# ShiveshM/GolemFlavor

Measured on AMD Instinct MI355X. Metric: walker-lnprob evals/sec (Gaussian llh, 100 walkers) at 1/2/4/8 MI355X, higher is better.
Workload: dtype f64

## Files before the change

### golemflavor_amd/csrc/gf_device.hpp

```cpp
#pragma once
#include <hip/hip_runtime.h>
#include <stdint.h>

#include "gf_consts.h"
#include "gf_elements.hpp"

#define GF_WAVE 64
#define GF_BLOCK 256
#define GF_WAVES_PER_BLOCK (GF_BLOCK / GF_WAVE)

#ifdef GF_COS_LITERALS
#define GF_COSC(c) nullptr
#else
#define GF_COSC(c) (c).cosc
#endif

namespace gfdev {

constexpr int ST_OK = 0, ST_OUT_OF_PRIOR = 1, ST_NON_UNITARY = 2, ST_NAN = 3;
constexpr int MODE_PRIOR_ONLY = 0, MODE_SM_GAUSS = 1, MODE_BSM_GAUSS = 2;
constexpr int MODE_BSM_BINNED = 3;
constexpr int MODE_BSM_TABLE = 4;

__device__ __forceinline__ double gf_inf() { return __longlong_as_double(0x7ff0000000000000LL); }
__device__ __forceinline__ double gf_nan() { return __longlong_as_double(0x7ff8000000000000LL); }


__device__ __forceinline__ double fast_sqrt(double x) { return gfel::el_sqrt(x); }

__device__ __forceinline__ double fast_rcp(double x)
{
    double r = __builtin_amdgcn_rcp(x);
    r = fma(fma(-x, r, 1.0), r, r);
    r = fma(fma(-x, r, 1.0), r, r);
    return r;
}

static __device__ __attribute__((noinline)) void sincos_cold(double x, double* sn, double* cs) { sincos(x, sn, cs); }

__device__ __forceinline__ void fast_sincos(double x, double* sn, double* cs)
{
    gfel::sincos_cw(x, sn, cs);
}

__device__ __forceinline__ double fast_cos(double x)
{
    double s, c;
    fast_sincos(x, &s, &c);
    return c;
}

static __device__ __attribute__((noinline)) double cos_general(double x) { return fast_cos(x); }

__device__ __forceinline__ double fast_cos_phase(double x, const double* k = nullptr)
{
    const double u = fabs(x - 3.141592653589793) - 1.5707963267948966;
    if (!(fabs(u) <= 1.5707963277948966)) return cos_general(x);
    const double z = u * u;
    double q;
    if (k) {
        q = fma(z, k[0], k[1]);
        q = fma(z, q, k[2]);
        q = fma(z, q, k[3]);
        q = fma(z, q, k[4]);
        q = fma(z, q, k[5]);
        q = fma(z, q, k[6]);
        q = fma(z, q, k[7]);
    } else {
        q = fma(z, 2.7117413873509064e-15, -7.641995277350052e-13);
        q = fma(z, q, 1.605889634387573e-10);
        q = fma(z, q, -2.505210587009456e-08);
        q = fma(z, q, 2.75573191979119e-06);
        q = fma(z, q, -0.00019841269841110079);
        q = fma(z, q, 0.008333333333332799);
        q = fma(z, q, -0.16666666666666657);
    }
    return fma(u * z, q, u);
}

__constant__ double GF_KTAB[26] = {
    2.7117413873509064e-15, -7.641995277350052e-13, 1.605889634387573e-10, -2.505210587009456e-08,
    2.75573191979119e-06, -0.00019841269841110079, 0.008333333333332799, -0.16666666666666657,
    4.695137892341541e-14, -1.1468837412893726e-11, 2.0876733673699156e-09, -2.755731905787651e-07,
    2.4801587300891894e-05, -0.0013888888888887252, 0.04166666666666665, -0.5,
    3.47933107596021167570e-05, 7.91534994289814532176e-04, -4.00555345006794114027e-02, 2.01212532134862925881e-01,
    -3.25565818622400915405e-01, 1.66666666666666657415e-01,
    7.70381505559019352791e-02, -6.88283971605453293030e-01, 2.02094576023350569471e+00, -2.40339491173441421878e+00};

__device__ __forceinline__ void sincos_small(double u, double* sn, double* cs)
{
    const double* k = GF_KTAB;
    const double z = u * u;
    double q = fma(z, k[0], k[1]);
    q = fma(z, q, k[2]);
    q = fma(z, q, k[3]);
    q = fma(z, q, k[4]);
    q = fma(z, q, k[5]);
    q = fma(z, q, k[6]);
    q = fma(z, q, k[7]);
    *sn = fma(u * z, q, u);
    double c = fma(z, k[8], k[9]);
    c = fma(z, c, k[10]);
    c = fma(z, c, k[11]);
    c = fma(z, c, k[12]);
    c = fma(z, c, k[13]);
    c = fma(z, c, k[14]);
    c = fma(z, c, k[15]);
    *cs = fma(z, c, 1.0);
}

__device__ __forceinline__ double fast_acos(double x)
{
    const double* k = GF_KTAB + 16;
    const double ax = fabs(x);
    const bool big = ax > 0.5;
    const double z = big ? fma(-0.5, ax, 0.5) : x * x;
    const double s = big ? fast_sqrt(z) : ax;
    double p = fma(z, k[0], k[1]);
    p = fma(z, p, k[2]);
    p = fma(z, p, k[3]);
    p = fma(z, p, k[4]);
    p = fma(z, p, k[5]);
    double q = fma(z, k[6], k[7]);
    q = fma(z, q, k[8]);
    q = fma(z, q, k[9]);
    q = fma(z, q, 1.0);
    const double r = (z * p) * fast_rcp(q);
    const double as = fma(s, r, s);
    const double a = big ? as + as : 1.5707963267948966 - as;
    return x < 0.0 ? 3.141592653589793 - a : a;
}

__device__ __forceinline__ double fast_acos_clamped(double x)
{
    const double* k = GF_KTAB + 16;
    const double ax = fabs(x);
    const bool big = ax > 0.5;
    const double z = big ? fmax(fma(-0.5, ax, 0.5), 0.0) : x * x;
    const double s = big ? fast_sqrt(z) : ax;
    double p = fma(z, k[0], k[1]);
    p = fma(z, p, k[2]);
    p = fma(z, p, k[3]);
    p = fma(z, p, k[4]);
// ... 6 lines not shown
    const double as = fma(s, r, s);
    const double a = big ? as + as : 1.5707963267948966 - as;
    return x < 0.0 ? 3.141592653589793 - a : a;
}

static __device__ __attribute__((noinline)) double pow10_cold(double x) { return pow(10.0, x); }
#ifdef GF_POW_LIBRARY
__device__ __forceinline__ double pow10_scale(double x) { return pow10_cold(x); }
#else
__constant__ double GF_P10TAB[18] = {
    3.321928094887362, 0.30102999560767785, 5.630334806675098e-11,
    1.3508629476223687e-06, 8.213412535439387e-06, 4.6371516642572196e-05, 0.00024166672554424694,
    0.0011544997789984348, 0.00501392883377544, 0.019597694626478524, 0.06808936507443707, 0.2069958486968681,
    0.5393829291955814, 1.171255148912267, 2.034678592293476, 2.650949055239199, 2.302585092994046, 1.0};
__device__ __forceinline__ double pow10_scale(double x)
{
    if (!(fabs(x) < 300.0)) return pow10_cold(x);
    const double* k = GF_P10TAB;
    const double n = rint(x * k[0]);
    double r = fma(-n, k[1], x);
    r = fma(-n, k[2], r);
    double p = k[3];
#pragma unroll
    for (int j = 4; j < 18; ++j) p = fma(p, r, k[j]);
    return ldexp(p, (int)n);
}
#endif

template <int NDIM>
__device__ __forceinline__ void stage_theta(const double* __restrict__ theta, int layout, int64_t n,
                                            int64_t w0, int ndim_rt, double* tile, int lane, int64_t n_stage = -1)
{
    const int ndim = NDIM ? NDIM : ndim_rt;
    const int64_t nlim = n_stage < 0 ? n : n_stage;
    const int64_t rows = (nlim - w0 < GF_WAVE) ? (nlim - w0) : GF_WAVE;
    if (layout == 0) {
        const int64_t count = rows * ndim;
        const double* src = theta + w0 * ndim;
        const int nvec = (GF_WAVE * ndim + 1) / 2;
#pragma unroll
        for (int j = 0; j < (NDIM ? (NDIM + 1) / 2 : (GF_MAX_DIM / 2)); ++j) {
            const int v = j * GF_WAVE + lane;
            if (!NDIM && v >= nvec) break;
            const int64_t d = 2 * (int64_t)v;
            if (d + 1 < count) {
                const double2 x = *reinterpret_cast<const double2*>(src + d);
                *reinterpret_cast<double2*>(tile + d) = x;
            } else if (d < count) {
                tile[d] = src[d];
            }
        }
    } else {
        if (lane < rows) {
#pragma unroll
            for (int d = 0; d < (NDIM ? NDIM : GF_MAX_DIM); ++d) {
                if (!NDIM && d >= ndim) break;
                tile[lane * ndim + d] = theta[(int64_t)d * n + w0 + lane];
            }
        }
    }
    __builtin_amdgcn_fence(__ATOMIC_RELEASE, "wavefront");
    __builtin_amdgcn_wave_barrier();
    __builtin_amdgcn_fence(__ATOMIC_ACQUIRE, "wavefront");
}

template <int NDIM>
__device__ __forceinline__ bool lnprior(const GfCommon& c, const double* row, double& lp)
{
    const int ndim = NDIM ? NDIM : c.ndim;
    bool inbox = true;
    double acc = 0.0;
#pragma unroll
    for (int d = 0; d < (NDIM ? NDIM : GF_MAX_DIM); ++d) {
        if (!NDIM && d >= ndim) break;
        const double x = row[d];
        inbox = inbox && (x >= c.lo[d]) && (x <= c.hi[d]);
        const double z = (x - c.loc[d]) * c.inv_sigma[d];
        acc = fma(-0.5 * z, z, acc);
    }
    lp = acc + c.prior_const;
    return inbox;
}

__device__ __forceinline__ void pmns_abs2(double s12_2, double c13_4, double s23_2, double dcp, double p[3][3],
                                          const double* cosc = nullptr)
{
    const double c13_2 = fast_sqrt(c13_4);
    const double s13_2 = 1.0 - c13_2;
    const double c12_2 = 1.0 - s12_2;
    const double c23_2 = 1.0 - s23_2;
    const double a = s12_2 * c23_2, b = c12_2 * s23_2;
    const double e = c12_2 * c23_2, f = s12_2 * s23_2;
    const double j2 = 2.0 * fast_sqrt((a * b) * s13_2) * fast_cos_phase(dcp, cosc);
    p[0][0] = c12_2 * c13_2;
    p[0][1] = s12_2 * c13_2;
    p[0][2] = s13_2;
    p[1][0] = fma(b, s13_2, a) + j2;
    p[1][1] = fma(f, s13_2, e) - j2;
    p[1][2] = s23_2 * c13_2;
}

using gfel::angles_to_fr;

__device__ __forceinline__ void propagate(const double p[3][3], const double src[3], double src_sum, double out[3])
{
    const double inv = fast_rcp(src_sum);
    const double s2 = src[2] * inv;
    const double ds0 = fma(src[0], inv, -s2), ds1 = fma(src[1], inv, -s2);
    const double w0 = fma(ds1, p[1][0], fma(ds0, p[0][0], s2));
    const double w1 = fma(ds1, p[1][1], fma(ds0, p[0][1], s2));
    const double w2 = fma(ds1, p[1][2], fma(ds0, p[0][2], s2));
    const double dw0 = w0 - w2, dw1 = w1 - w2;
    out[0] = fma(p[0][1], dw1, fma(p[0][0], dw0, w2));
    out[1] = fma(p[1][1], dw1, fma(p[1][0], dw0, w2));
    out[2] = (((w0 + w1) + w2) - out[0]) - out[1];
}

static __device__ __attribute__((noinline)) double log_of_exp_band(double x)
{
    const double HI = 744.4400719213812, LO = 4.422444340918698e-14;
    const double t = x + HI;
    const double y = exp(t) * (1.0 + LO);
    const double k = rint(y);
    if (!(k >= 1.0)) return (x != x) ? x : -gf_inf();
    return (log(k) - HI) - LO;
}

__device__ __forceinline__ double log_of_exp(double x, bool live = true)
{
    if (!live || x >= -708.3964185322641) return x;
    return log_of_exp_band(x);
}

__device__ __forceinline__ double gauss_llh(const GfCommon& c, const double fr[3], bool live = true)
{
    const double d0 = fr[0] - c.bf[0];
    const double d1 = fr[1] - c.bf[1];
    const double d2 = fr[2] - c.bf[2];
    const double r2 = fma(d2, d2, fma(d1, d1, d0 * d0));
    const double logpdf = fma(c.gauss_mh, r2, c.gauss_k);
    return log_of_exp(logpdf, live) + c.offset;
}

__device__ __forceinline__ double pick(const double* row, int idx, double fixed)
{
    return idx >= 0 ? row[idx] : fixed;
}

__device__ __forceinline__ void sm_composition(const GfCommon& c, const double* row, double fr[3])
{
    double p[3][3];
    pmns_abs2(pick(row, c.idx_sm[0], c.sm_fixed[0]), pick(row, c.idx_sm[1], c.sm_fixed[1]),
              pick(row, c.idx_sm[2], c.sm_fixed[2]), pick(row, c.idx_sm[3], c.sm_fixed[3]), p);
    double src[3], src_sum;
    if (c.idx_src[0] >= 0) {
        angles_to_fr(row[c.idx_src[0]], row[c.idx_src[1]], src);
        src_sum = (src[0] + src[1]) + src[2];
    } else if (c.idx_src_x >= 0) {
        const double x = row[c.idx_src_x], y = 1.0 - x;
        const double inv = fast_rcp((x + y) + 0.0);
        src[0] = x * inv; src[1] = y * inv; src[2] = 0.0;
        src_sum = (src[0] + src[1]) + src[2];
    } else {
        src[0] = c.src_fixed[0]; src[1] = c.src_fixed[1]; src[2] = c.src_fixed[2];
        src_sum = c.src_fixed_sum;
    }
    propagate(p, src, src_sum, fr);
}


template <int NDIM, int MODE, int SAMPLED, bool WANT_FR>
__device__ __forceinline__ void eval_walker(const GfCommon& c, const double* ctab, const double* row, int ndim_rt,
                                            double& val, double fr[3], int& st)
{
    const int ndim = NDIM ? NDIM : ndim_rt;
    bool inbox = true;
    double acc = 0.0;
#pragma unroll
    for (int d = 0; d < (NDIM ? NDIM : GF_MAX_DIM); ++d) {
        if (!NDIM && d >= ndim) break;
        const double x = row[d];
        const double2 lh = *reinterpret_cast<const double2*>(ctab + 4 * d);
        const double2 ls = *reinterpret_cast<const double2*>(ctab + 4 * d + 2);
        inbox = inbox & (x >= lh.x) & (x <= lh.y);
        const double z = (x - ls.x) * ls.y;
        acc = fma(-0.5 * z, z, acc);
#ifdef GF_DIM_BARRIER
        if ((d % GF_DIM_BARRIER) == GF_DIM_BARRIER - 1) __builtin_amdgcn_sched_barrier(0);
#endif
    }
    const double lp = acc + c.prior_const;
    double v;
    if (MODE == MODE_PRIOR_ONLY) {
        v = lp + c.flat_llh;
        if (WANT_FR) fr[0] = fr[1] = fr[2] = gf_nan();
    } else {
        double f[3];
        if (SAMPLED == 2) {
            double p[3][3], src[3];
            pmns_abs2(row[0], row[1], row[2], row[3], p, GF_COSC(c));
            angles_to_fr(row[4], row[5], src);
            propagate(p, src, (src[0] + src[1]) + src[2], f);
        } else if (SAMPLED == 1) {
            double p[3][3], src[3];
            pmns_abs2(row[c.idx_sm[0]], row[c.idx_sm[1]], row[c.idx_sm[2]], row[c.idx_sm[3]], p, GF_COSC(c));
            angles_to_fr(row[c.idx_src[0]], row[c.idx_src[1]], src);
            propagate(p, src, (src[0] + src[1]) + src[2], f);
        } else {
            sm_composition(c, row, f);
        }
        v = lp + gauss_llh(c, f, inbox);
        if (WANT_FR) {
            fr[0] = inbox ? f[0] : gf_nan(); fr[1] = inbox ? f[1] : gf_nan(); fr[2] = inbox ? f[2] : gf_nan();
        }
    }
    val = inbox ? v : -gf_inf();
    st = inbox ? ((v != v) ? ST_NAN : ST_OK) : ST_OUT_OF_PRIOR;
}


}
```

### golemflavor_amd/csrc/gf_propose.hpp

```cpp
#pragma once
#include <cstdlib>

#include "gf_device.hpp"
#include "gf_bsm_device.hpp"
#include "gf_launch.h"
#include "gf_table.hpp"

namespace {
using namespace gfdev;

__device__ __forceinline__ void philox_block(uint32_t c0, uint32_t c1, uint32_t c2, uint32_t c3, uint32_t k0,
                                             uint32_t k1, uint32_t out[4])
{
#pragma unroll
    for (int r = 0; r < 10; ++r) {
        const uint64_t m0 = (uint64_t)0xD2511F53u * c0;
        const uint64_t m1 = (uint64_t)0xCD9E8D57u * c2;
        const uint32_t n0 = __builtin_amdgcn_bitop3_b32((uint32_t)(m1 >> 32), c1, k0, 0x96);
        const uint32_t n1 = (uint32_t)m1;
        const uint32_t n2 = __builtin_amdgcn_bitop3_b32((uint32_t)(m0 >> 32), c3, k1, 0x96);
        const uint32_t n3 = (uint32_t)m0;
        c0 = n0; c1 = n1; c2 = n2; c3 = n3;
        k0 += 0x9E3779B9u; k1 += 0xBB67AE85u;
    }
    out[0] = c0; out[1] = c1; out[2] = c2; out[3] = c3;
}

template <int NDIM, int MODE, int LPW>
__device__ __forceinline__ double proposal_lnprob(const GfCommon& c, const GfBsm* tb, const double* ctab,
                                                  const double* ttab, const double* row, int ndim, int& st, int sub,
                                                  double* fgrp, unsigned long long& pending, const double* btab = nullptr,
                                                  int tside = 0)
{
    pending = 0ull;
    double val, fr[3];
    if constexpr (MODE == MODE_BSM_TABLE) {
        double lp;
        const bool inbox = lnprior_tab<NDIM>(ctab, row, ndim, c.prior_const, lp);
        asm volatile("" : "+v"(lp));
        val = -gf_inf();
        st = ST_OUT_OF_PRIOR;
        if (inbox) {
            UniAcc acc = {0.0, 0.0, 0ull, 2.0};
            flux_average<UNI_INLINE, LPW>(c, tb, ttab, row, fr, acc, sub, fgrp);
            st = (acc.clear_max < tb->uni_hi) ? ST_OK : ST_NON_UNITARY;
            pending = st == ST_OK ? uni_arbitration_mask(acc.amb, tb) : 0ull;
            val = lp + gftab::lookup(btab, tside, fr[0], fr[1]);
            if (val != val && st == ST_OK) st = ST_NAN;
        }
    } else if constexpr (MODE == MODE_BSM_BINNED || MODE == MODE_BSM_GAUSS) {
        static_assert(MODE != MODE_BSM_BINNED || LPW == 1, "the binned likelihood runs one lane per point");
        double lp;
        const bool inbox = lnprior_tab<NDIM>(ctab, row, ndim, c.prior_const, lp);
        asm volatile("" : "+v"(lp));
        val = -gf_inf();
        st = ST_OUT_OF_PRIOR;
        if (inbox) {
            UniAcc acc = {0.0, 0.0, 0ull, 2.0};
            double lnl = 0.0;
            if constexpr (MODE == MODE_BSM_BINNED) lnl = binned_llh<UNI_INLINE>(c, tb, ttab, btab, row, acc) + c.offset;
            else flux_average<UNI_INLINE, LPW>(c, tb, ttab, row, fr, acc, sub, fgrp);
            st = (acc.clear_max < tb->uni_hi) ? ST_OK : ST_NON_UNITARY;
            pending = st == ST_OK ? uni_arbitration_mask(acc.amb, tb) : 0ull;
            if constexpr (MODE != MODE_BSM_BINNED) lnl = gauss_llh(c, fr);
            val = lp + lnl;
            if (val != val && st == ST_OK) st = ST_NAN;
        }
    } else {
        eval_walker<NDIM, MODE, 0, false>(c, ctab, row, ndim, val, fr, st);
    }
    return val;
}

__device__ __forceinline__ void park_row(double* dst, const double* row, int ndim)
{
    for (int d = 0; d < ndim; ++d) dst[d] = row[d];
}

template <bool WITH_LHS = false>
__device__ __forceinline__ void park_proposal(GfArbQueue* pq, double* pend_rows, int64_t t, const double* row, int ndim, double lnq,
                                              unsigned long long pending, double lhs = 0.0)
{
    double* dst = pend_rows + (size_t)t * GF_PEND_STRIDE;
    park_row(dst, row, ndim);
    dst[GF_MAX_DIM] = lnq;
    if (WITH_LHS) dst[GF_MAX_DIM + 1] = lhs;
    const unsigned int at = atomicAdd(&pq->count, 1u);
    if (at < pq->cap) {
        GfArbItem it;
        it.walker = (unsigned long long)t;
        it.mask = pending;
        pq->items[at] = it;
    } else {
        pq->overflow = 1u;
    }
}

struct GfLpwRule {
    bool with2;
    size_t lds_cap;
    const char* force_env;
};
inline int lanes_per_walker(int mode, int64_t walkers, int nbins_max, int cus, const GfLpwRule& rule)
{
    if (mode != MODE_BSM_GAUSS || nbins_max < 2) return 1;
    const char* force = gf_internal_env(rule.force_env, 0);
    if (force) { const int f = std::atoi(force); if (f == 1 || (f == 2 && rule.with2) || f == 4 || f == 16) return f; }
    const int64_t simds = (int64_t)(cus > 0 ? cus : 256) * 4;
    int best = 1;
    double best_cost = 0.0;
    for (int lpw : {1, 2, 4, 16}) {
        if (lpw == 2 && !rule.with2) continue;
// ... 16 lines not shown
```

### golemflavor_amd/csrc/gf_sampler.hip

```cpp
#include <hip/hip_runtime.h>
#include <stdint.h>

#include <chrono>
#include <cstdio>
#include <cstdlib>
#include <cstring>
#include <cstddef>
#include <memory>
#include <new>

#include "gf_devcache.h"
#include "gf_host.h"
#include "gf_device.hpp"
#include "gf_bsm_device.hpp"
#include "gf_launch.h"
#include "gf_unitarity_teams.hpp"
#include "gf_propose.hpp"
#include "gf_stretch.hpp"

namespace {
using namespace gfdev;


struct StretchArgs {
// ... 102 lines not shown
        }
        s.lnp[wi] = lnq;
        s.naccept[wi] += 1u;
    }
    if (store_now) {
        double* dst = s.chain + (((int64_t)chain * s.nstore_cap + store_index) * s.nwalkers + w) * ndim;
#pragma unroll
        for (int d = 0; d < ND; ++d) {
            if (!NDIM && d >= ndim) break;
            dst[d] = accept ? row[d] : sk[d];
        }
        if (s.lnp_chain)
            s.lnp_chain[((int64_t)chain * s.nstore_cap + store_index) * s.nwalkers + w] = accept ? lnq : lnk;
    }
    }
}

#ifndef GF_STRETCH_WAVES
#define GF_STRETCH_WAVES 2
#endif
template <int NDIM, int MODE, int LPW>
__global__ __launch_bounds__(GF_BLOCK, GF_STRETCH_WAVES) void k_stretch(const GfCommon c, const GfBsm* __restrict__ tb,
                                                          const double* __restrict__ ptab, const StretchArgs s)
{
    const int nhalf = s.nwalkers / 2;
    const int64_t t = (int64_t)blockIdx.x * GF_BLOCK + threadIdx.x;
    const int64_t g = t / LPW;
    const bool valid = g < (int64_t)s.nchains * nhalf;
    const int chain = valid ? (int)(g / nhalf) : 0;
    const int k = valid ? (int)(g - (int64_t)chain * nhalf) : 0;
    if constexpr (MODE == MODE_BSM_BINNED) stretch_body<NDIM, MODE, LPW>(c, tb, ptab, s, chain, k, valid, 0, s.btabs[0]);
    else if constexpr (MODE == MODE_BSM_TABLE) stretch_body<NDIM, MODE, LPW>(c, tb, ptab, s, chain, k, valid, (int)(t % LPW), s.ttabs[0], s.tsides[0]);
    else stretch_body<NDIM, MODE, LPW>(c, tb, ptab, s, chain, k, valid, (int)(t % LPW));
}

template <int NDIM, int MODE, int LPW>
__global__ __launch_bounds__(GF_BLOCK, GF_STRETCH_WAVES) void k_stretch_multi(const StretchArgs s)
{
    const int chain = blockIdx.y;
    const int t = blockIdx.x * GF_BLOCK + threadIdx.x;
    const int k = t / LPW;
    if constexpr (MODE == MODE_BSM_BINNED)
        stretch_body<NDIM, MODE, LPW>(s.commons[chain], s.tbs[chain], s.ptabs[chain], s, chain, k, k < s.nwalkers / 2, 0, s.btabs[chain]);
    else if constexpr (MODE == MODE_BSM_TABLE)
        stretch_body<NDIM, MODE, LPW>(s.commons[chain], s.tbs[chain], s.ptabs[chain], s, chain, k, k < s.nwalkers / 2, t % LPW, s.ttabs[chain],
                                      s.tsides[chain]);
    else stretch_body<NDIM, MODE, LPW>(s.commons[chain], s.tbs[chain], s.ptabs[chain], s, chain, k, k < s.nwalkers / 2, t % LPW);
}

template <int NDIM, int MODE, int LPW>
hipError_t launch_stretch_nml(const GfCommon& c, const GfBsm* tb, const double* ptab, const StretchArgs& a, hipStream_t st)
{
    const size_t lds = LPW > 1 ? (size_t)(GF_BLOCK / LPW) * GF_FGRP_DOUBLES(a.nbins_max, LPW) * sizeof(double) : 0;
    if (a.commons) {
        const dim3 grid((unsigned)(((int64_t)(a.nwalkers / 2) * LPW + GF_BLOCK - 1) / GF_BLOCK), a.nchains);
        hipLaunchKernelGGL((k_stretch_multi<NDIM, MODE, LPW>), grid, dim3(GF_BLOCK), lds, st, a);
    } else {
        const int64_t total = (int64_t)a.nchains * (a.nwalkers / 2) * LPW;
        hipLaunchKernelGGL((k_stretch<NDIM, MODE, LPW>), dim3((unsigned)((total + GF_BLOCK - 1) / GF_BLOCK)), dim3(GF_BLOCK), lds, st,
                           c, tb, ptab, a);
    }
    return hipGetLastError();
}

struct PersistArgs {
    const GfCommon* commons;
    const double* const* ptabs;
    int32_t nmodels;
    int32_t nwalkers;
    double* pos;
    double* lnp;
    uint32_t* naccept;
    double* chain;
    double* lnp_chain;
    int64_t nstore_cap, store_base;
    uint64_t seed, iteration_base;
    int64_t nsteps;
    int32_t thin, store;
    double a;
    const uint64_t* stream_ids;
    int32_t workers;
};

template <int NDIM, int MODE, int MAXT>
__global__ __launch_bounds__(MAXT) void k_stretch_persist(const PersistArgs s)
{
    constexpr int ND = NDIM ? NDIM : GF_MAX_DIM;
    extern __shared__ __attribute__((aligned(16))) double dyn[];
    const int chain = blockIdx.x;
    const GfCommon& c = s.commons[s.nmodels > 1 ? chain : 0];
    const double* __restrict__ ptab = s.ptabs[s.nmodels > 1 ? chain : 0];
    const int ndim = NDIM ? NDIM : c.ndim;
    const int nw = s.nwalkers, nhalf = nw / 2, nt = blockDim.x;
    const int ntw = s.workers > 0 && s.workers < nt ? s.workers : nt;
    const int ntp = nt - ntw;
    const bool producer = (int)threadIdx.x >= ntw;
    double* ctab = dyn;
    double* pos = ctab + GF_MAX_DIM * 4;
    double* lnp = pos + (size_t)nw * ndim;
    double* rows = lnp + nw;
    uint32_t* nacc = reinterpret_cast<uint32_t*>(rows + (size_t)ntw * ndim);
    double* dz = reinterpret_cast<double*>(nacc + ((nw + 1) & ~1));
    double* dlhs = dz + 2 * (size_t)nhalf;
    int* dj = reinterpret_cast<int*>(dlhs + 2 * (size_t)nhalf);
    if (threadIdx.x < GF_MAX_DIM * 4) ctab[threadIdx.x] = ptab[threadIdx.x];
    const int64_t cw = (int64_t)chain * nw;
    for (int i = threadIdx.x; i < nw * ndim; i += nt) pos[i] = s.pos[cw * ndim + i];
    for (int i = threadIdx.x; i < nw; i += nt) { lnp[i] = s.lnp[cw + i]; nacc[i] = s.naccept[cw + i]; }
    double* row = rows + (size_t)(producer ? 0 : threadIdx.x) * ndim;
    const uint64_t gbase = (s.stream_ids ? s.stream_ids[chain] : (uint64_t)chain) * (uint64_t)nhalf;
    auto draw = [&](int k, uint64_t ctr, double& z, int& j, double& lhs) {
        double u3;
        stretch_draw(s.seed, gbase + (uint64_t)k, ctr, nhalf, s.a, z, j, u3);
        lhs = stretch_lhs(z, u3, ndim);
    };
    const uint64_t ctr_first = 2 * s.iteration_base, ctr_end = ctr_first + 2 * (uint64_t)s.nsteps;
    if (producer && s.nsteps > 0)
        for (int k = (int)threadIdx.x - ntw; k < nhalf; k += ntp) {
            double z, lhs; int j;
            draw(k, ctr_first, z, j, lhs);
            dz[k] = z; dlhs[k] = lhs; dj[k] = j;
        }
    __syncthreads();

    for (int64_t step = 0; step < s.nsteps; ++step) {
        const uint64_t iteration = s.iteration_base + (uint64_t)step;
        const bool store_now = s.store != 0 && s.chain != nullptr && (step % s.thin) == 0;
        const int64_t store_index = s.store_base + (step + s.thin - 1) / s.thin;
        for (int half = 0; half < 2; ++half) {
            const int cbase = (1 - half) * nhalf;
            const uint64_t ctr = 2 * iteration + half;
            const size_t buf = (size_t)(half) * nhalf;
            if (producer) {
                if (ctr + 1 < ctr_end)
                    for (int k = (int)threadIdx.x - ntw; k < nhalf; k += ntp) {
                        double z, lhs; int j;
                        draw(k, ctr + 1, z, j, lhs);
                        const size_t nb = (size_t)(1 - half) * nhalf;
                        dz[nb + k] = z; dlhs[nb + k] = lhs; dj[nb + k] = j;
                    }
            } else
            for (int k = threadIdx.x; k < nhalf; k += ntw) {
                const int w = half * nhalf + k;
                double z, lhs; int j;
                if (ntp > 0) { z = dz[buf + k]; lhs = dlhs[buf + k]; j = dj[buf + k]; }
                else draw(k, ctr, z, j, lhs);
                double* sk = pos + (size_t)w * ndim;
                const double* cj = pos + (size_t)(cbase + j) * ndim;
                stretch_row<NDIM>(row, cj, sk, z, ndim);
                int st;
                unsigned long long pending;
                const double lnq = proposal_lnprob<NDIM, MODE, 1>(c, nullptr, ctab, nullptr, row, ndim, st, 0, nullptr, pending);
                const double lnk = lnp[w];
                const bool accept = lhs > lnk - lnq;
                if (accept) {
#pragma unroll
                    for (int d = 0; d < ND; ++d) {
                        if (!NDIM && d >= ndim) break;
                        sk[d] = row[d];
                    }
                    lnp[w] = lnq;
                    nacc[w] += 1u;
                }
                if (store_now) {
                    double* dst = s.chain + (((int64_t)chain * s.nstore_cap + store_index) * nw + w) * ndim;
#pragma unroll
                    for (int d = 0; d < ND; ++d) {
                        if (!NDIM && d >= ndim) break;
                        dst[d] = sk[d];
                    }
                    if (s.lnp_chain) s.lnp_chain[((int64_t)chain * s.nstore_cap + store_index) * nw + w] = lnp[w];
                }
            }
            __syncthreads();
        }
    }
    for (int i = threadIdx.x; i < nw * ndim; i += nt) s.pos[cw * ndim + i] = pos[i];
    for (int i = threadIdx.x; i < nw; i += nt) { s.lnp[cw + i] = lnp[i]; s.naccept[cw + i] = nacc[i]; }
}

inline void persist_geometry(int nwalkers, int ndim, int* threads, size_t* lds, int* workers = nullptr, int nchains = 1, int cus = 256)
{
    const int nhalf = nwalkers / 2;
    int nt = ((nhalf + GF_WAVE - 1) / GF_WAVE) * GF_WAVE;
    if (nt > 512) nt = 512;
    static const bool no_producers = gf_internal_env("GF_SAMPLER_NO_PRODUCERS", 0) != nullptr;
    const size_t base = sizeof(double) * ((size_t)GF_MAX_DIM * 4 + (size_t)nwalkers * ndim + nwalkers + (size_t)nt * ndim) +
                        sizeof(uint32_t) * (size_t)((nwalkers + 1) & ~1);
    const size_t draws = (sizeof(double) * 4 + sizeof(int) * 2) * (size_t)nhalf;
    const bool producers = nt <= 256 && !no_producers && base + draws <= 64 * 1024 && nchains <= 2 * cus;
    const size_t bytes = base + (producers ? draws : 0);
    if (workers) *workers = nt;
    *threads = producers ? 2 * nt : nt;
    *lds = (bytes <= 64 * 1024 && nhalf <= 4 * 1024) ? bytes : 0;
}

template <int NDIM>
hipError_t launch_persist_n(int mode, int nchains, int threads, size_t lds, const PersistArgs& a, hipStream_t st)
{
    if (mode == MODE_PRIOR_ONLY) {
        if (threads <= 256) hipLaunchKernelGGL((k_stretch_persist<NDIM, MODE_PRIOR_ONLY, 256>), dim3(nchains), dim3(threads), lds, st, a);
        else hipLaunchKernelGGL((k_stretch_persist<NDIM, MODE_PRIOR_ONLY, 512>), dim3(nchains), dim3(threads), lds, st, a);
    } else {
        if (threads <= 256) hipLaunchKernelGGL((k_stretch_persist<NDIM, MODE_SM_GAUSS, 256>), dim3(nchains), dim3(threads), lds, st, a);
        else hipLaunchKernelGGL((k_stretch_persist<NDIM, MODE_SM_GAUSS, 512>), dim3(nchains), dim3(threads), lds, st, a);
    }
    return hipGetLastError();
}

hipError_t launch_persist(int mode, int ndim, int nchains, int threads, size_t lds, const PersistArgs& a, hipStream_t st)
{
    switch (ndim) {
    case 4: return launch_persist_n<4>(mode, nchains, threads, lds, a, st);
    case 6: return launch_persist_n<6>(mode, nchains, threads, lds, a, st);
    case 7: return launch_persist_n<7>(mode, nchains, threads, lds, a, st);
    case 12: return launch_persist_n<12>(mode, nchains, threads, lds, a, st);
    default: return launch_persist_n<0>(mode, nchains, threads, lds, a, st);
    }
}

struct ChainArgs {
    const GfCommon* commons;
    const GfBsm* const* tbs;
    const GfBsm* tb;
    const double* const* ptabs;
    int32_t nmodels;
    int32_t nwalkers;
    double* pos;
    double* lnp;
    uint32_t* naccept;
    uint32_t* flags;
    double* pend_rows;
    double* chain;
    double* lnp_chain;
    int64_t nstore_cap, store_base;
    uint64_t seed, iteration_base;
    int64_t run_step_base;
    int32_t nsteps, thin, store;
    double a;
    const uint64_t* stream_ids;
    double* lazy_rows;
    unsigned long long* lazy_mask;
    int32_t lazy_cap;
    unsigned long long* stats;
};

constexpr int CH_BLOCK = 512;
constexpr int CH_WAVES = CH_BLOCK / GF_WAVE;

typedef __attribute__((address_space(3))) double* LdsD;
typedef __attribute__((address_space(3))) unsigned int* LdsU;
typedef __attribute__((address_space(3))) int* LdsI;
typedef __attribute__((address_space(3))) unsigned long long* LdsL;

template <int NDIM>
__device__ __attribute__((noinline)) void chain_propose(const ChainArgs& s, const GfCommon& c, const GfBsm* __restrict__ tb, LdsD ctab_l, LdsD ttab_l,
                                                        LdsD row_l, const int chain, const int k, const int half, const uint64_t iteration,
                                                        const bool store_now, const int64_t store_index, const uint64_t sid, double* my_pend,
                                                        double* lz_rows, unsigned long long* lz_mask, LdsU pk_n, LdsI pk_k, LdsL pk_mask, LdsU lz_n)
{
    constexpr int ND = NDIM ? NDIM : GF_MAX_DIM;
    const double* ctab = (const double*)ctab_l;
    const double* ttab = (const double*)ttab_l;
    double* row = (double*)row_l;
    const int ndim = NDIM ? NDIM : c.ndim;
    const int nw = s.nwalkers, nhalf = nw / 2;
    const int cbase = (1 - half) * nhalf;
    const uint64_t g = sid * (uint64_t)nhalf + (uint64_t)k;
    const int w = half * nhalf + k;
    double z, u3;
    int j;
    stretch_draw(s.seed, g, 2 * iteration + half, nhalf, s.a, z, j, u3);
    const int64_t wi = (int64_t)chain * nw + w;
    const double* sk = s.pos + wi * ndim;
    const double* cj = s.pos + ((int64_t)chain * nw + cbase + j) * ndim;
#pragma unroll
    for (int d = 0; d < ND; ++d) {
        if (!NDIM && d >= ndim) break;
        const double cv = cj[d];
        row[d] = fma(-z, cv - sk[d], cv);
    }
    int st;
    unsigned long long pending;
    const double lnq = proposal_lnprob<NDIM, MODE_BSM_GAUSS, 1>(c, tb, ctab, ttab, row, ndim, st, 0, nullptr, pending);
    const double lnk = s.lnp[wi];
    const double lhs = stretch_lhs(z, u3, ndim);
    bool accept = lhs > lnk - lnq;
    if (pending != 0ull && accept) {
        double* dst = my_pend + (size_t)k * GF_PEND_STRIDE;
        park_row(dst, row, ndim);
        dst[GF_MAX_DIM] = lnq;
        dst[GF_MAX_DIM + 1] = lhs;
        const unsigned int at = atomicAdd((unsigned int*)pk_n, 1u);
        pk_k[at] = k;
        pk_mask[at] = pending;
    } else {
        if (pending != 0ull) {
            const unsigned int at = atomicAdd((unsigned int*)lz_n, 1u);
            park_row(lz_rows + (size_t)at * GF_PEND_STRIDE, row, ndim);
            lz_mask[at] = pending;
        }
// ... 996 lines not shown
    s->steps_since_reset += nsteps;
    s->nstored += nstore;
    return GF_OK;
}

int gf_sampler_sync(gf_sampler* s)
{
    if (!s) return GF_ERR_INVALID_ARG;
    return gf_model_sync(s->model);
}

int gf_sampler_run_to_host(gf_sampler* s, int64_t nsteps, int thin, double* chain, double* lnprob_chain, double* readback_tail_s)
{
    if (!s || !chain || nsteps < 0 || thin < 1) return GF_ERR_INVALID_ARG;
    GF_HIP(hipSetDevice(s->device));
    const int device = s->device;
    void* copy_stream = nullptr;
    int rc = gf_internal_borrow_copy_stream(device, &copy_stream);
    if (rc != GF_OK) return rc;
    HostSink sink;
    sink.chain = chain; sink.lnp = lnprob_chain; sink.total = s->nstored + (nsteps + thin - 1) / thin;
    sink.copy_stream = copy_stream; sink.device = device;
    sink.last_event = sink.t_entry = std::chrono::steady_clock::now();
    if (gf_internal_env("GF_RUN_TO_HOST_NO_PIPE", 0) == nullptr) {
        rc = gf_internal_d2h_pipe_open(device, copy_stream, &sink.pipe);
        if (rc != GF_OK) { gf_internal_return_copy_stream(device, copy_stream); return rc; }
    }
    const bool marks = gf_internal_env("GF_RUN_TO_HOST_NO_MARKS", 0) == nullptr;
    s->sink = marks ? &sink : nullptr;
    rc = gf_sampler_run(s, nsteps, thin, 1);
    hipError_t e = hipSuccess;
    while (rc == GF_OK && e == hipSuccess && s->flight_done < s->flight_enq) e = flight_consume(s, true);
    s->sink = nullptr;
    const hipError_t e2 = hipStreamSynchronize(s->stream);
    auto t_done = marks && s->flight_enq > 0 ? sink.last_event : std::chrono::steady_clock::now();
    if (rc == GF_OK && e == hipSuccess && e2 == hipSuccess && sink.rc == GF_OK) {
        s->sink = &sink;
        (void)sink_copy(s, s->nstored);
        s->sink = nullptr;
    }
    const int rc_pipe = gf_internal_d2h_pipe_close(sink.pipe);
    (void)hipStreamSynchronize((hipStream_t)copy_stream);
    gf_internal_return_copy_stream(device, copy_stream);
    if (rc == GF_OK && sink.rc == GF_OK) sink.rc = rc_pipe;
    if (readback_tail_s) *readback_tail_s = std::chrono::duration<double>(std::chrono::steady_clock::now() - t_done).count();
    for (int i = 0; i < 8; ++i) g_last_run_to_host_times[i] = sink.t[i];
    if (rc != GF_OK) return rc;
    if (sink.rc != GF_OK) return sink.rc;
    if (e == hipSuccess) e = e2;
    if (e != hipSuccess) return gf_hip_fail(e, "gf_sampler_run_to_host");
    return GF_OK;
}

int gf_internal_sampler_chain_stats(gf_sampler* s, unsigned long long* out)
{
    if (!s || !out) return GF_ERR_INVALID_ARG;
    if (!s->d_chain_stats) return GF_ERR_UNSUPPORTED;
    GF_HIP(hipSetDevice(s->device));
    GF_HIP(hipMemcpyAsync(out, s->d_chain_stats, sizeof(unsigned long long) * 8 * (size_t)s->nchains, hipMemcpyDeviceToHost, s->stream));
    GF_HIP(hipStreamSynchronize(s->stream));
    return GF_OK;
}

int gf_internal_run_to_host_times(double out[8])
{
    if (!out) return GF_ERR_INVALID_ARG;
    for (int i = 0; i < 8; ++i) out[i] = g_last_run_to_host_times[i];
    return GF_OK;
}
int gf_internal_run_prologue_times(double out[4])
{
    if (!out) return GF_ERR_INVALID_ARG;
    for (int i = 0; i < 4; ++i) out[i] = g_last_run_prologue[i];
    return GF_OK;
}

int gf_internal_sampler_shape(const gf_sampler* s, double out[3])
{
    if (!s || !out) return GF_ERR_INVALID_ARG;
    out[0] = (double)s->shape; out[1] = s->probe_us[0]; out[2] = s->probe_us[1];
    return GF_OK;
}

int64_t gf_sampler_nstored(const gf_sampler* s) { return s ? s->nstored : -1; }
int64_t gf_sampler_iterations(const gf_sampler* s) { return s ? s->steps_since_reset : -1; }

int gf_internal_sampler_chain_view(const gf_sampler* s, GfChainView* v)
{
    if (!s || !v) return GF_ERR_INVALID_ARG;
    *v = GfChainView{s->device, s->stream, s->cus, s->nchains, s->nwalkers, s->ndim, s->nstored, s->nstore_cap, s->d_chain, s->model, s->models,
                     s->d_lnp_chain, s->seed, s->d_stream_ids};
    return GF_OK;
}

int gf_sampler_get_state(gf_sampler* s, double* pos, double* lnprob)
{
    if (!s) return GF_ERR_INVALID_ARG;
    int rc = gf_model_sync(s->model);
    if (rc != GF_OK) return rc;
    GF_HIP(hipSetDevice(s->device));
    const size_t nw = (size_t)s->nchains * s->nwalkers;
    hipStream_t st = s->stream;
    if (pos) GF_HIP(hipMemcpyAsync(pos, s->d_pos, sizeof(double) * nw * s->ndim, hipMemcpyDeviceToHost, st));
    if (lnprob) GF_HIP(hipMemcpyAsync(lnprob, s->d_lnp, sizeof(double) * nw, hipMemcpyDeviceToHost, st));
    GF_HIP(hipStreamSynchronize(st));
    return GF_OK;
}

int gf_sampler_get_chain(gf_sampler* s, double* chain, double* lnprob_chain, uint32_t* naccepted, uint32_t* nonunitary)
{
    if (!s) return GF_ERR_INVALID_ARG;
    GF_HIP(hipSetDevice(s->device));
    hipStream_t st = s->stream;
    const size_t per = (size_t)s->nwalkers;
    if (s->nstored > 0) {
        const size_t row = sizeof(double) * per * s->ndim, lrow = sizeof(double) * per;
        if (chain) {
            const int rc = gf_internal_d2h_2d(s->device, st, chain, row * s->nstored, s->d_chain, row * s->nstore_cap, row * s->nstored,
                                              (size_t)s->nchains);
            if (rc != GF_OK) return rc;
        }
        if (lnprob_chain) {
            const int rc = gf_internal_d2h_2d(s->device, st, lnprob_chain, lrow * s->nstored, s->d_lnp_chain, lrow * s->nstore_cap,
                                              lrow * s->nstored, (size_t)s->nchains);
            if (rc != GF_OK) return rc;
        }
    }
    if (naccepted)
        GF_HIP(hipMemcpyAsync(naccepted, s->d_naccept, sizeof(uint32_t) * (size_t)s->nchains * per, hipMemcpyDeviceToHost, st));
    if (nonunitary) GF_HIP(hipMemcpyAsync(nonunitary, s->d_flags, sizeof(uint32_t), hipMemcpyDeviceToHost, st));
    GF_HIP(hipStreamSynchronize(st));
    return GF_OK;
}

int gf_sampler_get_chain_device(gf_sampler* s, double* d_chain, double* d_lnprob_chain)
{
    if (!s) return GF_ERR_INVALID_ARG;
    GF_HIP(hipSetDevice(s->device));
    hipStream_t st = s->stream;
    if (s->nstored > 0) {
        const size_t row = sizeof(double) * (size_t)s->nwalkers * s->ndim, lrow = sizeof(double) * (size_t)s->nwalkers;
        if (d_chain)
            GF_HIP(hipMemcpy2DAsync(d_chain, row * s->nstored, s->d_chain, row * s->nstore_cap, row * s->nstored, s->nchains,
                                     hipMemcpyDeviceToDevice, st));
        if (d_lnprob_chain)
            GF_HIP(hipMemcpy2DAsync(d_lnprob_chain, lrow * s->nstored, s->d_lnp_chain, lrow * s->nstore_cap, lrow * s->nstored,
                                     s->nchains, hipMemcpyDeviceToDevice, st));
    }
    GF_HIP(hipStreamSynchronize(st));
    return GF_OK;
}

hipError_t gf_launch_walker_mean(const double* d_chain, int64_t cap, int64_t nstored, int nchains, int nwalkers, int ndim, double* d_mean,
                                 hipStream_t st)
{
    hipError_t e = hipSuccess;
    for (int ch0 = 0; ch0 < nchains && e == hipSuccess; ch0 += 65535) {
        const int nch = nchains - ch0 < 65535 ? nchains - ch0 : 65535;
        hipLaunchKernelGGL(k_walker_mean, dim3((unsigned)nstored, (unsigned)nch), dim3(GF_BLOCK), 0, st,
                           d_chain + (size_t)ch0 * cap * nwalkers * ndim, cap, nstored, nwalkers, ndim, d_mean + (size_t)ch0 * nstored * ndim);
        e = hipGetLastError();
    }
    return e;
}

int gf_sampler_walker_mean(gf_sampler* s, double* mean)
// ... 19 lines not shown
```

Baseline: 106.1 billion.

## Stage persistent-kernel constants in LDS and raise waves-per-EU launch bounds

The persistent stretch kernel now copies the per-chain model constants, seed, output pointers and chain-store bases into a shared-memory struct once per block. The inner loop reads from that struct through templated likelihood helpers, with 32-bit indexing and incremental store counters, and launch bounds request 4 waves per EU for small NDIM. The aim is to cut SGPR/VGPR pressure and 64-bit address arithmetic so more waves can be resident and scalar loads drop. In exchange it uses more LDS per block, risks spills under the tighter register cap, and adds a diagnostic resource-query entry point.

```diff
diff --git a/golemflavor_amd/csrc/gf_device.hpp b/golemflavor_amd/csrc/gf_device.hpp
--- a/golemflavor_amd/csrc/gf_device.hpp
+++ b/golemflavor_amd/csrc/gf_device.hpp
@@ -52,13 +52,14 @@
 
 static __device__ __attribute__((noinline)) double cos_general(double x) { return fast_cos(x); }
 
+template <bool TABLE = false>
 __device__ __forceinline__ double fast_cos_phase(double x, const double* k = nullptr)
 {
     const double u = fabs(x - 3.141592653589793) - 1.5707963267948966;
     if (!(fabs(u) <= 1.5707963277948966)) return cos_general(x);
     const double z = u * u;
     double q;
-    if (k) {
+    if (TABLE || k) {
         q = fma(z, k[0], k[1]);
         q = fma(z, q, k[2]);
         q = fma(z, q, k[3]);
@@ -231,6 +232,7 @@
     return inbox;
 }
 
+template <bool TABLE = false>
 __device__ __forceinline__ void pmns_abs2(double s12_2, double c13_4, double s23_2, double dcp, double p[3][3],
                                           const double* cosc = nullptr)
 {
@@ -240,7 +242,7 @@
     const double c23_2 = 1.0 - s23_2;
     const double a = s12_2 * c23_2, b = c12_2 * s23_2;
     const double e = c12_2 * c23_2, f = s12_2 * s23_2;
-    const double j2 = 2.0 * fast_sqrt((a * b) * s13_2) * fast_cos_phase(dcp, cosc);
+    const double j2 = 2.0 * fast_sqrt((a * b) * s13_2) * fast_cos_phase<TABLE>(dcp, cosc);
     p[0][0] = c12_2 * c13_2;
     p[0][1] = s12_2 * c13_2;
     p[0][2] = s13_2;
@@ -281,7 +283,8 @@
     return log_of_exp_band(x);
 }
 
-__device__ __forceinline__ double gauss_llh(const GfCommon& c, const double fr[3], bool live = true)
+template <class C>
+__device__ __forceinline__ double gauss_llh(const C& c, const double fr[3], bool live = true)
 {
     const double d0 = fr[0] - c.bf[0];
     const double d1 = fr[1] - c.bf[1];
@@ -296,11 +299,23 @@
     return idx >= 0 ? row[idx] : fixed;
 }
 
-__device__ __forceinline__ void sm_composition(const GfCommon& c, const double* row, double fr[3])
+template <class C>
+struct SmCosc {
+    static constexpr bool table = true;
+    static __device__ __forceinline__ const double* of(const C& c) { return c.cosc; }
+};
+template <>
+struct SmCosc<GfCommon> {
+    static constexpr bool table = false;
+    static __device__ __forceinline__ const double* of(const GfCommon&) { return nullptr; }
+};
+
+template <class C>
+__device__ __forceinline__ void sm_composition(const C& c, const double* row, double fr[3])
 {
     double p[3][3];
-    pmns_abs2(pick(row, c.idx_sm[0], c.sm_fixed[0]), pick(row, c.idx_sm[1], c.sm_fixed[1]),
-              pick(row, c.idx_sm[2], c.sm_fixed[2]), pick(row, c.idx_sm[3], c.sm_fixed[3]), p);
+    pmns_abs2<SmCosc<C>::table>(pick(row, c.idx_sm[0], c.sm_fixed[0]), pick(row, c.idx_sm[1], c.sm_fixed[1]),
+                                pick(row, c.idx_sm[2], c.sm_fixed[2]), pick(row, c.idx_sm[3], c.sm_fixed[3]), p, SmCosc<C>::of(c));
     double src[3], src_sum;
     if (c.idx_src[0] >= 0) {
         angles_to_fr(row[c.idx_src[0]], row[c.idx_src[1]], src);
@@ -318,8 +333,8 @@
 }
 
 
-template <int NDIM, int MODE, int SAMPLED, bool WANT_FR>
-__device__ __forceinline__ void eval_walker(const GfCommon& c, const double* ctab, const double* row, int ndim_rt,
+template <int NDIM, int MODE, int SAMPLED, bool WANT_FR, class C>
+__device__ __forceinline__ void eval_walker(const C& c, const double* ctab, const double* row, int ndim_rt,
                                             double& val, double fr[3], int& st)
 {
     const int ndim = NDIM ? NDIM : ndim_rt;
diff --git a/golemflavor_amd/csrc/gf_propose.hpp b/golemflavor_amd/csrc/gf_propose.hpp
--- a/golemflavor_amd/csrc/gf_propose.hpp
+++ b/golemflavor_amd/csrc/gf_propose.hpp
@@ -26,8 +26,8 @@
     out[0] = c0; out[1] = c1; out[2] = c2; out[3] = c3;
 }
 
-template <int NDIM, int MODE, int LPW>
-__device__ __forceinline__ double proposal_lnprob(const GfCommon& c, const GfBsm* tb, const double* ctab,
+template <int NDIM, int MODE, int LPW, class C>
+__device__ __forceinline__ double proposal_lnprob(const C& c, const GfBsm* tb, const double* ctab,
                                                   const double* ttab, const double* row, int ndim, int& st, int sub,
                                                   double* fgrp, unsigned long long& pending, const double* btab = nullptr,
                                                   int tside = 0)
diff --git a/golemflavor_amd/csrc/gf_sampler.hip b/golemflavor_amd/csrc/gf_sampler.hip
--- a/golemflavor_amd/csrc/gf_sampler.hip
+++ b/golemflavor_amd/csrc/gf_sampler.hip
@@ -208,75 +208,148 @@
     int32_t workers;
 };
 
+struct PersistConsts {
+    double prior_const, flat_llh;
+    double sm_fixed[4];
+    double src_fixed[3];
+    double src_fixed_sum;
+    double bf[3];
+    double gauss_mh, gauss_k, offset;
+    int32_t idx_sm[4];
+    int32_t idx_src[2];
+    int32_t idx_src_x, ndim;
+    double cosc[8];
+    double a;
+    uint32_t seed[2];
+    uint64_t gbase;
+    double* out_pos;
+    double* out_lnp;
+    uint32_t* out_naccept;
+    double* chain0;
+    double* lnp_chain0;
+};
+constexpr int PERSIST_CONSTS_DOUBLES = (int)((sizeof(PersistConsts) + 15) / 16) * 2;
+
+__device__ __forceinline__ void persist_consts_fill(PersistConsts* k, const GfCommon* __restrict__ c, double a, uint64_t seed)
+{
+    k->a = a; k->seed[0] = (uint32_t)seed; k->seed[1] = (uint32_t)(seed >> 32);
+    k->prior_const = c->prior_const; k->flat_llh = c->flat_llh;
+    for (int i = 0; i < 4; ++i) { k->sm_fixed[i] = c->sm_fixed[i]; k->idx_sm[i] = c->idx_sm[i]; }
+    for (int i = 0; i < 3; ++i) { k->src_fixed[i] = c->src_fixed[i]; k->bf[i] = c->bf[i]; }
+    k->src_fixed_sum = c->src_fixed_sum;
+    k->gauss_mh = c->gauss_mh; k->gauss_k = c->gauss_k; k->offset = c->offset;
+    k->idx_src[0] = c->idx_src[0]; k->idx_src[1] = c->idx_src[1]; k->idx_src_x = c->idx_src_x; k->ndim = c->ndim;
+    for (int i = 0; i < 8; ++i) k->cosc[i] = c->cosc[i];
+}
+
+template <int NDIM>
+static __device__ __attribute__((noinline)) double persist_lhs(double z, double u3, int ndim_rt)
+{
+    return stretch_lhs(z, u3, NDIM ? NDIM : ndim_rt);
+}
+
 template <int NDIM, int MODE, int MAXT>
-__global__ __launch_bounds__(MAXT) void k_stretch_persist(const PersistArgs s)
+constexpr int persist_waves_per_eu()
+{
+#ifdef GF_PERSIST_THREE_WAVES
+    return MAXT == 256 && (NDIM == 4 || NDIM == 6 || NDIM == 7) ? 3 : (MAXT == 512 ? 2 : 1);
+#else
+    return MAXT == 256 && (NDIM == 4 || NDIM == 6 || NDIM == 7) ? 4 : (MAXT == 512 ? 2 : 1);
+#endif
+}
+
+template <int NDIM, int MODE, int MAXT>
+__global__ __launch_bounds__(MAXT, (persist_waves_per_eu<NDIM, MODE, MAXT>())) void k_stretch_persist(const PersistArgs s)
 {
     constexpr int ND = NDIM ? NDIM : GF_MAX_DIM;
     extern __shared__ __attribute__((aligned(16))) double dyn[];
+#ifdef GF_PERSIST_THREE_WAVES
+    if constexpr (persist_waves_per_eu<NDIM, MODE, MAXT>() == 3) asm volatile("" ::: "v135");
+#endif
     const int chain = blockIdx.x;
-    const GfCommon& c = s.commons[s.nmodels > 1 ? chain : 0];
+    const GfCommon* __restrict__ cg = s.commons + (s.nmodels > 1 ? chain : 0);
     const double* __restrict__ ptab = s.ptabs[s.nmodels > 1 ? chain : 0];
-    const int ndim = NDIM ? NDIM : c.ndim;
+    const int ndim = NDIM ? NDIM : cg->ndim;
     const int nw = s.nwalkers, nhalf = nw / 2, nt = blockDim.x;
     const int ntw = s.workers > 0 && s.workers < nt ? s.workers : nt;
     const int ntp = nt - ntw;
     const bool producer = (int)threadIdx.x >= ntw;
     double* ctab = dyn;
-    double* pos = ctab + GF_MAX_DIM * 4;
-    double* lnp = pos + (size_t)nw * ndim;
+    PersistConsts* kc = reinterpret_cast<PersistConsts*>(ctab + GF_MAX_DIM * 4);
+    double* pos = ctab + GF_MAX_DIM * 4 + PERSIST_CONSTS_DOUBLES;
+    double* lnp = pos + nw * ndim;
     double* rows = lnp + nw;
-    uint32_t* nacc = reinterpret_cast<uint32_t*>(rows + (size_t)ntw * ndim);
+    uint32_t* nacc = reinterpret_cast<uint32_t*>(rows + ntw * ndim);
     double* dz = reinterpret_cast<double*>(nacc + ((nw + 1) & ~1));
-    double* dlhs = dz + 2 * (size_t)nhalf;
-    int* dj = reinterpret_cast<int*>(dlhs + 2 * (size_t)nhalf);
+    double* dlhs = dz + 2 * nhalf;
+    int* dj = reinterpret_cast<int*>(dlhs + 2 * nhalf);
     if (threadIdx.x < GF_MAX_DIM * 4) ctab[threadIdx.x] = ptab[threadIdx.x];
-    const int64_t cw = (int64_t)chain * nw;
-    for (int i = threadIdx.x; i < nw * ndim; i += nt) pos[i] = s.pos[cw * ndim + i];
-    for (int i = threadIdx.x; i < nw; i += nt) { lnp[i] = s.lnp[cw + i]; nacc[i] = s.naccept[cw + i]; }
-    double* row = rows + (size_t)(producer ? 0 : threadIdx.x) * ndim;
-    const uint64_t gbase = (s.stream_ids ? s.stream_ids[chain] : (uint64_t)chain) * (uint64_t)nhalf;
-    auto draw = [&](int k, uint64_t ctr, double& z, int& j, double& lhs) {
+    {
+        const int64_t cw = (int64_t)chain * nw;
+        double* gpos = s.pos + cw * ndim;
+        double* glnp = s.lnp + cw;
+        uint32_t* gnacc = s.naccept + cw;
+        if (threadIdx.x == 0) {
+            persist_consts_fill(kc, cg, s.a, s.seed);
+            kc->gbase = (s.stream_ids ? s.stream_ids[chain] : (uint64_t)chain) * (uint64_t)nhalf;
+            kc->out_pos = gpos; kc->out_lnp = glnp; kc->out_naccept = gnacc;
+            const int64_t first = ((int64_t)chain * s.nstore_cap + s.store_base) * nw;
+            kc->chain0 = s.chain ? s.chain + first * ndim : nullptr;
+            kc->lnp_chain0 = s.lnp_chain ? s.lnp_chain + first : nullptr;
+        }
+        for (int i = threadIdx.x; i < nw * ndim; i += nt) pos[i] = gpos[i];
+        for (int i = threadIdx.x; i < nw; i += nt) { lnp[i] = glnp[i]; nacc[i] = gnacc[i]; }
+    }
+    auto draw = [&](int k, uint64_t ctr, double& z, int& j, double& lhs, int ndim) {
         double u3;
-        stretch_draw(s.seed, gbase + (uint64_t)k, ctr, nhalf, s.a, z, j, u3);
-        lhs = stretch_lhs(z, u3, ndim);
+        const uint32_t seed_lo = (uint32_t)__builtin_amdgcn_readfirstlane(kc->seed[0]), seed_hi = (uint32_t)__builtin_amdgcn_readfirstlane(kc->seed[1]);
+        const uint64_t seed = (uint64_t)seed_hi << 32 | seed_lo;
+        stretch_draw(seed, kc->gbase + (uint64_t)k, ctr, nhalf, kc->a, z, j, u3);
+        lhs = persist_lhs<NDIM>(z, u3, ndim);
     };
-    const uint64_t ctr_first = 2 * s.iteration_base, ctr_end = ctr_first + 2 * (uint64_t)s.nsteps;
-    if (producer && s.nsteps > 0)
+    const int nsteps = (int)s.nsteps;
+    uint64_t ctr = 2 * s.iteration_base;
+    __syncthreads();
+    if (producer && nsteps > 0)
         for (int k = (int)threadIdx.x - ntw; k < nhalf; k += ntp) {
             double z, lhs; int j;
-            draw(k, ctr_first, z, j, lhs);
+            draw(k, ctr, z, j, lhs, ndim);
             dz[k] = z; dlhs[k] = lhs; dj[k] = j;
         }
     __syncthreads();
 
-    for (int64_t step = 0; step < s.nsteps; ++step) {
-        const uint64_t iteration = s.iteration_base + (uint64_t)step;
-        const bool store_now = s.store != 0 && s.chain != nullptr && (step % s.thin) == 0;
-        const int64_t store_index = s.store_base + (step + s.thin - 1) / s.thin;
-        for (int half = 0; half < 2; ++half) {
-            const int cbase = (1 - half) * nhalf;
-            const uint64_t ctr = 2 * iteration + half;
-            const size_t buf = (size_t)(half) * nhalf;
+    int until_store = s.store != 0 && s.chain != nullptr ? 0 : 1 << 30;
+    uint32_t srow = 0;
+    for (int step = 0; step < nsteps; ++step) {
+        const bool store_now = until_store == 0;
+        for (int half = 0; half < 2; ++half, ++ctr) {
+            const int hoff = half ? nhalf : 0;
+            const int coff = nhalf - hoff;
             if (producer) {
-                if (ctr + 1 < ctr_end)
-                    for (int k = (int)threadIdx.x - ntw; k < nhalf; k += ntp) {
+                if (half == 0 || step + 1 < nsteps)
+                    for (int kl = (int)threadIdx.x - ntw; kl < nhalf; kl += ntp) {
+                        int k = kl;
+                        asm volatile("" : "+v"(k));
                         double z, lhs; int j;
-                        draw(k, ctr + 1, z, j, lhs);
-                        const size_t nb = (size_t)(1 - half) * nhalf;
-                        dz[nb + k] = z; dlhs[nb + k] = lhs; dj[nb + k] = j;
+                        draw(k, ctr + 1, z, j, lhs, ndim);
+                        dz[coff + k] = z; dlhs[coff + k] = lhs; dj[coff + k] = j;
                     }
             } else
-            for (int k = threadIdx.x; k < nhalf; k += ntw) {
-                const int w = half * nhalf + k;
+            for (int kl = threadIdx.x; kl < nhalf; kl += ntw) {
+                int k = kl;
+                asm volatile("" : "+v"(k));
+                const int ndim = NDIM ? NDIM : __builtin_amdgcn_readfirstlane(kc->ndim);
+                const int w = hoff + k;
                 double z, lhs; int j;
-                if (ntp > 0) { z = dz[buf + k]; lhs = dlhs[buf + k]; j = dj[buf + k]; }
-                else draw(k, ctr, z, j, lhs);
-                double* sk = pos + (size_t)w * ndim;
-                const double* cj = pos + (size_t)(cbase + j) * ndim;
+                if (ntp > 0) { z = dz[w]; lhs = dlhs[w]; j = dj[w]; }
+                else draw(k, ctr, z, j, lhs, ndim);
+                double* row = rows + (int)threadIdx.x * ndim;
+                double* sk = pos + w * ndim;
+                const double* cj = pos + (coff + j) * ndim;
                 stretch_row<NDIM>(row, cj, sk, z, ndim);
                 int st;
                 unsigned long long pending;
-                const double lnq = proposal_lnprob<NDIM, MODE, 1>(c, nullptr, ctab, nullptr, row, ndim, st, 0, nullptr, pending);
+                const double lnq = proposal_lnprob<NDIM, MODE, 1>(*kc, nullptr, ctab, nullptr, row, ndim, st, 0, nullptr, pending);
                 const double lnk = lnp[w];
                 const bool accept = lhs > lnk - lnq;
                 if (accept) {
@@ -289,20 +362,32 @@
                     nacc[w] += 1u;
                 }
                 if (store_now) {
-                    double* dst = s.chain + (((int64_t)chain * s.nstore_cap + store_index) * nw + w) * ndim;
+                    const uint32_t e = srow + (uint32_t)w;
+                    double* dst = kc->chain0 + (uint64_t)e * (uint32_t)ndim;
 #pragma unroll
                     for (int d = 0; d < ND; ++d) {
                         if (!NDIM && d >= ndim) break;
                         dst[d] = sk[d];
                     }
-                    if (s.lnp_chain) s.lnp_chain[((int64_t)chain * s.nstore_cap + store_index) * nw + w] = lnp[w];
+                    double* ldst = kc->lnp_chain0;
+                    if (ldst) ldst[e] = lnp[w];
                 }
             }
             __syncthreads();
         }
-    }
-    for (int i = threadIdx.x; i < nw * ndim; i += nt) s.pos[cw * ndim + i] = pos[i];
-    for (int i = threadIdx.x; i < nw; i += nt) { s.lnp[cw + i] = lnp[i]; s.naccept[cw + i] = nacc[i]; }
+        if (store_now) {
+            srow += (uint32_t)nw;
+            until_store = s.thin;
+        }
+        --until_store;
+    }
+    double* gpos = kc->out_pos;
+    double* glnp = kc->out_lnp;
+    uint32_t* gnacc = kc->out_naccept;
+    int t0 = threadIdx.x;
+    asm volatile("" : "+v"(t0));
+    for (int i = t0; i < nw * ndim; i += nt) gpos[i] = pos[i];
+    for (int i = t0; i < nw; i += nt) { glnp[i] = lnp[i]; gnacc[i] = nacc[i]; }
 }
 
 inline void persist_geometry(int nwalkers, int ndim, int* threads, size_t* lds, int* workers = nullptr, int nchains = 1, int cus = 256)
@@ -310,8 +395,8 @@
     const int nhalf = nwalkers / 2;
     int nt = ((nhalf + GF_WAVE - 1) / GF_WAVE) * GF_WAVE;
     if (nt > 512) nt = 512;
-    static const bool no_producers = gf_internal_env("GF_SAMPLER_NO_PRODUCERS", 0) != nullptr;
-    const size_t base = sizeof(double) * ((size_t)GF_MAX_DIM * 4 + (size_t)nwalkers * ndim + nwalkers + (size_t)nt * ndim) +
+    const bool no_producers = gf_internal_env("GF_SAMPLER_NO_PRODUCERS", 0) != nullptr;
+    const size_t base = sizeof(double) * ((size_t)GF_MAX_DIM * 4 + PERSIST_CONSTS_DOUBLES + (size_t)nwalkers * ndim + nwalkers + (size_t)nt * ndim) +
                         sizeof(uint32_t) * (size_t)((nwalkers + 1) & ~1);
     const size_t draws = (sizeof(double) * 4 + sizeof(int) * 2) * (size_t)nhalf;
     const bool producers = nt <= 256 && !no_producers && base + draws <= 64 * 1024 && nchains <= 2 * cus;
@@ -321,28 +406,29 @@
     *lds = (bytes <= 64 * 1024 && nhalf <= 4 * 1024) ? bytes : 0;
 }
 
+using PersistKernel = void (*)(const PersistArgs);
 template <int NDIM>
-hipError_t launch_persist_n(int mode, int nchains, int threads, size_t lds, const PersistArgs& a, hipStream_t st)
-{
-    if (mode == MODE_PRIOR_ONLY) {
-        if (threads <= 256) hipLaunchKernelGGL((k_stretch_persist<NDIM, MODE_PRIOR_ONLY, 256>), dim3(nchains), dim3(threads), lds, st, a);
-        else hipLaunchKernelGGL((k_stretch_persist<NDIM, MODE_PRIOR_ONLY, 512>), dim3(nchains), dim3(threads), lds, st, a);
-    } else {
-        if (threads <= 256) hipLaunchKernelGGL((k_stretch_persist<NDIM, MODE_SM_GAUSS, 256>), dim3(nchains), dim3(threads), lds, st, a);
-        else hipLaunchKernelGGL((k_stretch_persist<NDIM, MODE_SM_GAUSS, 512>), dim3(nchains), dim3(threads), lds, st, a);
-    }
+PersistKernel persist_kernel_n(int mode, int threads)
+{
+    if (mode == MODE_PRIOR_ONLY) return threads <= 256 ? k_stretch_persist<NDIM, MODE_PRIOR_ONLY, 256> : k_stretch_persist<NDIM, MODE_PRIOR_ONLY, 512>;
+    return threads <= 256 ? k_stretch_persist<NDIM, MODE_SM_GAUSS, 256> : k_stretch_persist<NDIM, MODE_SM_GAUSS, 512>;
+}
+
+PersistKernel persist_kernel(int mode, int ndim, int threads)
+{
+    switch (ndim) {
+    case 4: return persist_kernel_n<4>(mode, threads);
+    case 6: return persist_kernel_n<6>(mode, threads);
+    case 7: return persist_kernel_n<7>(mode, threads);
+    case 12: return persist_kernel_n<12>(mode, threads);
+    default: return persist_kernel_n<0>(mode, threads);
+    }
+}
+
+hipError_t launch_persist(int mode, int ndim, int nchains, int threads, size_t lds, const PersistArgs& a, hipStream_t st)
+{
+    hipLaunchKernelGGL(persist_kernel(mode, ndim, threads), dim3(nchains), dim3(threads), lds, st, a);
     return hipGetLastError();
-}
-
-hipError_t launch_persist(int mode, int ndim, int nchains, int threads, size_t lds, const PersistArgs& a, hipStream_t st)
-{
-    switch (ndim) {
-    case 4: return launch_persist_n<4>(mode, nchains, threads, lds, a, st);
-    case 6: return launch_persist_n<6>(mode, nchains, threads, lds, a, st);
-    case 7: return launch_persist_n<7>(mode, nchains, threads, lds, a, st);
-    case 12: return launch_persist_n<12>(mode, nchains, threads, lds, a, st);
-    default: return launch_persist_n<0>(mode, nchains, threads, lds, a, st);
-    }
 }
 
 struct ChainArgs {
@@ -1505,6 +1591,26 @@
     return GF_OK;
 }
 
+int gf_internal_persist_resources(int ndim, int mode, int nwalkers, int nchains, int64_t out[4])
+{
+    if (!out || ndim < 1 || ndim > GF_MAX_DIM || (mode != MODE_PRIOR_ONLY && mode != MODE_SM_GAUSS) || nwalkers < 2 || nchains < 1)
+        return GF_ERR_INVALID_ARG;
+    int device = 0, cus = 0;
+    GF_HIP(hipGetDevice(&device));
+    GF_HIP(hipDeviceGetAttribute(&cus, hipDeviceAttributeMultiprocessorCount, device));
+    int threads = 0;
+    size_t lds = 0;
+    persist_geometry(nwalkers, ndim, &threads, &lds, nullptr, nchains, cus);
+    if (lds == 0) return GF_ERR_UNSUPPORTED;
+    const void* k = reinterpret_cast<const void*>(persist_kernel(mode, ndim, threads));
+    hipFuncAttributes fa;
+    GF_HIP(hipFuncGetAttributes(&fa, k));
+    int blocks = 0;
+    GF_HIP(hipOccupancyMaxActiveBlocksPerMultiprocessor(&blocks, k, threads, lds));
+    out[0] = fa.numRegs; out[1] = (int64_t)fa.localSizeBytes; out[2] = (int64_t)lds; out[3] = blocks;
+    return GF_OK;
+}
+
 int64_t gf_sampler_nstored(const gf_sampler* s) { return s ? s->nstored : -1; }
 int64_t gf_sampler_iterations(const gf_sampler* s) { return s ? s->steps_since_reset : -1; }
 
```

Result: slower. 98.98 billion (-6.7%).
